# mmurooka/SMPLpp

Hardware: AMD Instinct MI355X
Metric: SMPL FK evals/s + IK iters/s, batch 1024 frames, 1/2/4/8 MI355X (higher is better)
Workload: dtype f32 (exact operands: every fp32 value as three bf16 pieces = fp32's 24 bits on the bf16 matrix pipe, fp32 accumulate; fp32 VALU skinning)

## Files before the change

### smplpp_amd/csrc/ik.hip

```cpp
#include "ik_types.h"
#include "ik_eval.h"
#include "ik_solve.h"
#include "ik_proj.h"
#include "vposer_state.h"

#include <algorithm>
#include <chrono>
#include <cstdlib>

using namespace smplpp_hip;

struct smplpp_ik
{
  smplpp_model * m = nullptr;
  smplpp_vposer * vp = nullptr;
  int64_t n = 0, K = 0;
  int64_t frame_base = 0;
  int theta_dim = TD75;
  TaskArrays ta{};
  float *theta = nullptr, *beta = nullptr, *theta25 = nullptr, *vjac = nullptr;
  float *verts = nullptr, *rest = nullptr, *joints = nullptr, *poserot = nullptr, *pts = nullptr;
  double *e = nullptr, *J = nullptr, *Jl = nullptr, *e2 = nullptr, *xout = nullptr;
  int *skip = nullptr, *status = nullptr, *sticky = nullptr, *list_cnt = nullptr, *list_f = nullptr;
  int * range_word = nullptr;
// ... 343 lines not shown
    HIP_TRY(hipDeviceSynchronize());
    HIP_TRY(hipMemcpy(actual_normal, s->ta.anrm, sizeof(float) * nk * 3, kind));
  }
  return SMPLPP_OK;
}

static int ik_forward_eval(smplpp_ik * s, int optimize_beta, int phi_live, int64_t min_valid, hipStream_t st, hipEvent_t eval_done = nullptr)
{
  smplpp_model * m = s->m;
  const int64_t n = s->n;
  const int K = (int)s->K;
  const float * th25 = s->theta;
  const bool jac_elsewhere = s->vp && s->jac_ahead;
  {
    TraceRange tr_fwd("forward SMPL");
    if(s->vp && s->exact)
    {
      int rc = vposer_jacobian_device(s->vp, s->jxw, n, s->theta + 6, TD44, s->theta25 + 6, 75, s->vjac, st);
      if(rc) return rc;
      th25 = s->theta25;
    }
    else if(s->vp)
    {
      int rc = jac_elsewhere ? vposer_forward_device(s->vp, n, s->theta + 6, TD44, s->theta25 + 6, 75, nullptr, st, s->frame_base, true)
                             : vposer_forward_device(s->vp, n, s->theta + 6, TD44, s->theta25 + 6, 75, s->vjac, st, s->frame_base);
      if(rc) return rc;
      th25 = s->theta25;
    }
    s->vcur ^= 1;
    s->verts = s->vbuf[s->vcur];
    int rc = fk_device(m, n, s->beta, th25, s->verts, s->joints, nullptr, s->rest, s->poserot, st, RANGE_INTERNAL, s->range_word,
                       s->exact ? m->form : 0);
    if(rc) return rc;
  }
  TraceRange tr_eval("calculate IK matrices");
  if(s->side_pending)
  {
    if(s->use_flags)
      HIP_TRY(hipStreamWaitValue32(st, s->sig + 32, s->tick_join, hipStreamWaitValueGte, 0xffffffffu));
    else
      HIP_TRY(hipStreamWaitEvent(st, s->ev_join, 0));
    s->side_pending = false;
  }
  s->jac_ahead = false;
  const bool deep = m->nlev > 9;
  const bool wide = m->madj > MAXADJ;
  const size_t shmem = sizeof(float) * (deep ? (wide ? EvalPlan<DMAX, 64, 3>::L_END : EvalPlan<DMAX, 64, 3>::L_END)
                                             : (wide ? EvalPlan<9, 76, 4>::L_END : EvalPlan<9, 76, 6>::L_END)) + L_ANC_BYTES;
  static PerDeviceOnce once_eval[4];
  const void * kfn = deep ? (wide ? reinterpret_cast<const void *>(&ik_eval_kernel<DMAX, 64, 3, MAXADJ_WIDE>) : reinterpret_cast<const void *>(&ik_eval_kernel<DMAX, 64, 3>))
                          : (wide ? reinterpret_cast<const void *>(&ik_eval_kernel<9, 76, 4, MAXADJ_WIDE>) : reinterpret_cast<const void *>(&ik_eval_kernel<9, 76, 6>));
  HIP_TRY(lds_opt_in(once_eval[(deep ? 1 : 0) + (wide ? 2 : 0)], m->device, kfn, (int)shmem));
  int tsplit = (n < 256) ? (int)(256 / n) : 1;
  if(tsplit > K) tsplit = K;
  if(tsplit < 1) tsplit = 1;
  if(s->use_flags) eval_done = nullptr;
#define EVAL_(DM, RC, NG, MA)                                                                                                              \
  hipExtLaunchKernelGGL((ik_eval_kernel<DM, RC, NG, MA>), dim3((unsigned)(n * tsplit)), dim3(EVAL_NT), shmem, st, nullptr, eval_done, 0,     \
                        view_of(m), s->ta, th25, (const float *)s->verts, (const float *)s->rest, (const float *)m->ws.Gp.as<float>(),     \
                        (const float *)s->joints, (const float *)s->poserot, K, optimize_beta, phi_live, (int)min_valid, s->pts, s->e,     \
                        s->J, s->skip, s->dbg_stop, tsplit, s->roles, s->vp ? (const float *)s->vjac : (const float *)nullptr,             \
                        s->vp ? s->Jl : (double *)nullptr)
  if(deep && wide)
    EVAL_(DMAX, 64, 3, MAXADJ_WIDE);
  else if(deep)
    EVAL_(DMAX, 64, 3, MAXADJ);
  else if(wide)
    EVAL_(9, 76, 4, MAXADJ_WIDE);
  else
    EVAL_(9, 76, 6, MAXADJ);
#undef EVAL_
  HIP_TRY(hipGetLastError());
  s->have_eval = true;
  return SMPLPP_OK;
}

static int ik_check_valence(smplpp_ik * s);

extern "C" int smplpp_ik_eval(smplpp_ik * s, int optimize_beta, double * e, double * J, int space, void * stream)
{
  if(!s) return fail(SMPLPP_ERR_INVALID, "smplpp_ik_eval: null solver");
  int rc = check_space(space, "smplpp_ik_eval");
  if(rc) return rc;
  HIP_TRY(hipSetDevice(s->m->device));
  hipStream_t st = static_cast<hipStream_t>(stream);
  rc = ik_forward_eval(s, optimize_beta, 1, 0, st);
  if(rc) return rc;
  const int64_t D = s->theta_dim + 2 * s->K + (optimize_beta ? NB : 0);
  hipMemcpyKind kind = space == SMPLPP_HOST ? hipMemcpyDeviceToHost : hipMemcpyDeviceToDevice;
  if(e) HIP_TRY(hipMemcpyAsync(e, s->e, sizeof(double) * s->n * s->K * 4, kind, st));
  if(J) HIP_TRY(hipMemcpyAsync(J, s->vp ? s->Jl : s->J, sizeof(double) * s->n * s->K * 4 * D, kind, st));
  if(space == SMPLPP_HOST)
  {
    HIP_TRY(hipStreamSynchronize(st));
    if((rc = ik_check_valence(s))) return rc;
  }
  return SMPLPP_OK;
}

struct SeqHook
{
  float * theta_record = nullptr;
  const float * next_tpos = nullptr;
  const uint8_t * next_valid = nullptr;
  int shared = 0;
};

static int ik_iterate_enqueue(smplpp_ik * s, int iters, int enable_qp, int optimize_beta_from, int64_t min_valid, hipStream_t st,
                              const SeqHook * hook = nullptr, bool more_follows = false)
{
  int rc = SMPLPP_OK;
  smplpp_model * m = s->m;
  const int K = (int)s->K;
  static PerDeviceOnce once_solve[5];
  HIP_TRY(lds_opt_in(once_solve[0], m->device, reinterpret_cast<const void *>(&ik_solve_kernel<false>), (int)SOLVE_LDS_MAX));
  HIP_TRY(lds_opt_in(once_solve[1], m->device, reinterpret_cast<const void *>(&ik_solve_kernel<true>), (int)SOLVE_LDS_MAX));
  HIP_TRY(lds_opt_in(once_solve[2], m->device, reinterpret_cast<const void *>(&ik_solve_kernel<false, 11>), (int)SOLVE_LDS_MAX));
  HIP_TRY(lds_opt_in(once_solve[3], m->device, reinterpret_cast<const void *>(&ik_solve_kernel<false, 5>), (int)SOLVE_LDS_MAX));
  HIP_TRY(lds_opt_in(once_solve[4], m->device, reinterpret_cast<const void *>(&ik_solve_kernel<false, 3>), (int)SOLVE_LDS_MAX));
  if(s->use_flags && (s->tick_fork > 0x7fff0000u || s->tick_join > 0x7fff0000u || s->tick_done > 0x7fff0000u))
  {
    HIP_TRY(hipStreamSynchronize(st));
    HIP_TRY(hipStreamSynchronize(s->side));
    HIP_TRY(hipMemset(s->sig, 0, sizeof(unsigned) * 128));
    s->tick_fork = s->tick_join = s->tick_done = 0;
  }
  const bool dbg = s->dbg_sync;
  const int dbg_stop = s->dbg_stop;
  const bool overlap_ok = s->overlap_ok;
  const int64_t scan_blocks = s->scan_blocks;
#define DBG_SYNC(tag)                                                            \
  if(dbg)                                                                        \
  {                                                                              \
    fprintf(stderr, "[smplpp dbg] it %d: %s ...\n", it, tag);                    \
    HIP_TRY(hipStreamSynchronize(st));                                           \
    fprintf(stderr, "[smplpp dbg] it %d: %s done\n", it, tag);                   \
  }
  for(int it = 0; it < iters; it++)
  {
    const int opt_beta = (optimize_beta_from >= 0 && it >= optimize_beta_from) ? 1 : 0;
    const int phi_live = (optimize_beta_from >= 0) ? (it >= optimize_beta_from ? 1 : 0) : 1;
    const bool beside = overlap_ok && (!phi_live || s->phi_locked);
    rc = ik_forward_eval(s, opt_beta, phi_live, min_valid, st, beside ? s->ev_fork : nullptr);
    if(rc) return rc;
    DBG_SYNC("forward+eval");
    const int beta_dim = opt_beta ? NB : 0;
    const int D = s->theta_dim + 2 * K + beta_dim, rows = 4 * K;
    s->last_D = D;
    const int m_dim = D - ((!phi_live || s->phi_locked) ? 2 * K : 0);
    const int qp_k = (enable_qp && !((!phi_live || s->phi_locked) && beta_dim == 0)) ? 1 : 0;
    const int ntr_primal = (m_dim + 1 <= 48) ? 3 : (m_dim + 1 <= 80) ? 5 : ((m_dim + 1 <= 96 || m_dim + 1 > 176) ? 6 : 11);
    const bool dual_shape = rows < s->theta_dim && rows <= 63 && D <= 192 && dbg_stop != 9;
    const int ntr = dual_shape ? 6 : ntr_primal;
    const size_t fixed = sizeof(double) * ((size_t)(m_dim + 1) * (m_dim + 2) / 2 + 7 * (size_t)D + 2 * (size_t)rows + 128 * (size_t)ntr + 4) + sizeof(int) * 2 * (size_t)D;
    const size_t budget = SOLVE_LDS_MAX;
    int chunk_rows = (int)((budget - fixed) / (sizeof(double) * (size_t)D));
    if(chunk_rows > rows) chunk_rows = rows;
    if(chunk_rows < 4) return fail(SMPLPP_ERR_INVALID, "smplpp_ik_iterate: system too large for the in-LDS solver");
    const size_t solve_shmem = fixed + sizeof(double) * (size_t)chunk_rows * D;
    const bool dual_only = dual_shape && chunk_rows >= rows;
    if(dual_shape && !dual_only) return fail(SMPLPP_ERR_INVALID, "smplpp_ik_iterate: system too large for the in-LDS solver");
    const bool last = hook && it == iters - 1;
    float * theta_record = last ? hook->theta_record : nullptr;
    const bool go = beside && s->use_flags;
    if(go) s->tick_fork++;
    const bool ahead = s->latent_split && go && !opt_beta && (it + 1 < iters || more_follows);
    if(ahead) s->tick_done++;
    unsigned * const done_flag = ahead ? s->sig + 64 : (unsigned *)nullptr;
    unsigned * const done_counter = ahead ? s->sig + 80 : (unsigned *)nullptr;
#define SOLVE_(DO) ik_solve_kernel<DO><<<dim3((unsigned)s->n), dim3(256), solve_shmem, st>>>(                                              \
    s->ta, s->e, s->vp ? s->Jl : s->J, s->theta, s->beta, beside ? nullptr : s->pts, K, s->theta_dim, beta_dim, phi_live, qp_k, \
    s->vp ? 1 : 0, chunk_rows, s->skip, s->e2, s->status, s->sticky, s->xout, dbg_stop, m_dim, s->vp ? s->theta25 : (float *)nullptr, theta_record, \
    go ? s->sig : (unsigned *)nullptr, go ? s->sig + 16 : (unsigned *)nullptr, s->tick_fork, done_flag, done_counter, s->tick_done)
#define SOLVE11_(NTR_) ik_solve_kernel<false, NTR_><<<dim3((unsigned)s->n), dim3(256), solve_shmem, st>>>(                                              \
    s->ta, s->e, s->vp ? s->Jl : s->J, s->theta, s->beta, beside ? nullptr : s->pts, K, s->theta_dim, beta_dim, phi_live, qp_k, \
    s->vp ? 1 : 0, chunk_rows, s->skip, s->e2, s->status, s->sticky, s->xout, dbg_stop, m_dim, s->vp ? s->theta25 : (float *)nullptr, theta_record, \
    go ? s->sig : (unsigned *)nullptr, go ? s->sig + 16 : (unsigned *)nullptr, s->tick_fork, done_flag, done_counter, s->tick_done)
    {
      TraceRange tr_solve("solve IK");
      if(dual_only)
        SOLVE_(true);
      else if(ntr == 11)
        SOLVE11_(11);
      else if(ntr == 5)
        SOLVE11_(5);
      else if(ntr == 3)
        SOLVE11_(3);
      else
        SOLVE_(false);
    }
#undef SOLVE_
#undef SOLVE11_
    HIP_TRY(hipGetLastError());
    DBG_SYNC("solve");
    {
      TraceRange tr_proj("project point");
      const float * qpts = beside ? s->ta.apos : s->pts;
      hipStream_t pst = st;
      if(beside)
      {
        if(s->use_flags)
          HIP_TRY(hipStreamWaitValue32(s->side, s->sig, s->tick_fork, hipStreamWaitValueGte, 0xffffffffu));
        else
          HIP_TRY(hipStreamWaitEvent(s->side, s->ev_fork, 0));
        pst = s->side;
      }
      int chunks = (int)(scan_blocks / s->n);
      chunks = chunks < 1 ? 1 : (chunks > 32 ? 32 : chunks);
      const float * hint = beside ? s->ta.hint : nullptr;
      const dim3 sg((unsigned)(s->n * chunks));
#define SCAN_(KPR, NBT_) proj_scan_kernel<KPR, NBT_><<<sg, dim3(256), 0, pst>>>(view_of(m), s->ta, s->verts, qpts, hint, m->F, K, chunks, s->skip, \
                                                                   s->list_cnt, s->list_d, s->list_f, dbg_stop)
      const bool small_chunk = (m->F + chunks - 1) / chunks <= 3 * 256;
      const bool many = s->scan_form < 0 ? (s->n >= 512 && small_chunk) : s->scan_form == 0;
      if(K <= 8 && many && small_chunk) SCAN_(0, 3);
      else if(K <= 8 && many) SCAN_(0, CP_BATCH);
      else if(K <= 4) SCAN_(2, CP_BATCH);
      else if(K <= 8) SCAN_(4, CP_BATCH);
      else if(small_chunk) SCAN_(0, 3);
      else SCAN_(0, CP_BATCH);
#undef SCAN_
      HIP_TRY(hipGetLastError());
      int *& dbg_buf = s->dbg_buf;
      if(dbg && !dbg_buf) HIP_TRY(dalloc(s, &dbg_buf, 8));
      if(dbg) HIP_TRY(hipMemsetAsync(dbg_buf, 0, sizeof(int) * 8, st));
      int fsplit = (s->n < 256) ? (int)(256 / s->n) : 1;
      if(fsplit > K) fsplit = K;
      if(fsplit < 1) fsplit = 1;
      const bool join_flag = beside && s->use_flags && !ahead;
      if(beside && s->use_flags) s->tick_join++;
      hipExtLaunchKernelGGL(proj_finish_kernel, dim3((unsigned)(s->n * fsplit)), dim3(256), 0, pst, nullptr,
                            (beside && !s->use_flags) ? s->ev_join : nullptr, 0,
                            view_of(m), s->ta, (const float *)s->verts, qpts, m->F, K, (const int *)s->skip, s->list_cnt, s->list_d,
                            s->list_f, dbg ? dbg_buf : (int *)nullptr, fsplit, join_flag ? s->sig + 32 : (unsigned *)nullptr,
                            join_flag ? s->sig + 48 : (unsigned *)nullptr, s->tick_join, last ? hook->next_tpos : (const float *)nullptr,
                            last ? hook->next_valid : (const uint8_t *)nullptr, last ? hook->shared : 0);
      HIP_TRY(hipGetLastError());
      if(ahead)
      {
        HIP_TRY(hipStreamWaitValue32(s->side, s->sig + 64, s->tick_done, hipStreamWaitValueGte, 0xffffffffu));
        rc = vposer_forward_device(s->vp, s->n, s->theta + 6, TD44, nullptr, 75, s->vjac, s->side, s->frame_base, false, s->sig + 32,
                                   s->sig + 48, s->tick_join);
        if(rc) return rc;
        s->jac_ahead = true;
      }
      if(beside) s->side_pending = true;
      if(dbg)
      {
        int h[8];
        HIP_TRY(hipMemcpy(h, dbg_buf, sizeof(h), hipMemcpyDeviceToHost));
        fprintf(stderr, "[smplpp dbg] it %d: project lists: tasks %d, empty %d, overflow %d, nan %d, max cnt %d\n", it, h[0], h[1], h[2], h[3], h[4]);
      }
    }
    DBG_SYNC("project");
  }
#undef DBG_SYNC
  return SMPLPP_OK;
}

static int ik_join(smplpp_ik * s, hipStream_t st)
{
  if(s->side_pending)
  {
    if(s->use_flags)
      HIP_TRY(hipStreamWaitValue32(st, s->sig + 32, s->tick_join, hipStreamWaitValueGte, 0xffffffffu));
    else
      HIP_TRY(hipStreamWaitEvent(st, s->ev_join, 0));
    s->side_pending = false;
  }
  return SMPLPP_OK;
}

static int ik_check_status(smplpp_ik * s, const int * flags)
{
  std::vector<int> h((size_t)s->n);
  HIP_TRY(hipMemcpy(h.data(), flags, sizeof(int) * s->n, hipMemcpyDeviceToHost));
  for(int64_t f = 0; f < s->n; f++)
    if(h[f] & 1) return fail(SMPLPP_ERR_NUMERIC, "LLT has numerical issue!");
  return SMPLPP_OK;
}

static int ik_check_valence(smplpp_ik * s)
{
  std::vector<int> h((size_t)s->n);
  HIP_TRY(hipMemcpy(h.data(), s->sticky, sizeof(int) * s->n, hipMemcpyDeviceToHost));
  for(int64_t f = 0; f < s->n; f++)
    if(h[f] & 4)
      return fail(SMPLPP_ERR_INVALID, "a task with a normal term (normal weight or normal offset) touches a vertex with more than 12 adjacent "
                                      "faces: the Jacobian of such a term is not supported");
  return SMPLPP_OK;
}

extern "C" int smplpp_ik_iterate(smplpp_ik * s, int iters, int enable_qp, int optimize_beta_from, int64_t min_valid,
                                 double * e_sqnorm, int space, void * stream)
{
  if(!s || iters < 0) return fail(SMPLPP_ERR_INVALID, "smplpp_ik_iterate: bad argument");
  int rc = check_space(space, "smplpp_ik_iterate");
  if(rc) return rc;
  HIP_TRY(hipSetDevice(s->m->device));
  hipStream_t st = static_cast<hipStream_t>(stream);
  const auto enq_t0 = std::chrono::steady_clock::now();
  rc = ik_iterate_enqueue(s, iters, enable_qp, optimize_beta_from, min_valid, st);
  s->last_enqueue_us = std::chrono::duration<double, std::micro>(std::chrono::steady_clock::now() - enq_t0).count();
  if(rc)
  {
    (void)ik_join(s, st);
    return rc;
// ... 162 lines not shown
```

### smplpp_amd/csrc/ik_solve.h

```cpp
#pragma once
#include "ik_types.h"

namespace smplpp_hip
{
__device__ inline int tri_idx(int i, int j)
{
  return i * (i + 1) / 2 + j;
}
__device__ inline void tri_unpack(int item, int & i, int & j)
{
  i = (int)((sqrt(8.0 * (double)item + 1.0) - 1.0) * 0.5);
  while(tri_idx(i + 1, 0) <= item) i++;
  while(tri_idx(i, 0) > item) i--;
  j = item - tri_idx(i, 0);
}

__device__ inline void chol_aug(double * M, int nf, int * bad, double * dinv)
{
  const int tid = threadIdx.x, nt = blockDim.x;
  for(int j = 0; j < nf; j++)
  {
    double d = M[tri_idx(j, j)];
    if(!(d > 0.0))
    {
// ... 250 lines not shown
      for(; m + 1 < k; m += 2)
      {
        s -= Li[m] * Lk[m];
        s1 -= Li[m + 1] * Lk[m + 1];
      }
      if(m < k) s -= Li[m] * Lk[m];
      s += s1;
    }
    double piv = readlane_f64(s, k);
    if(!(piv > 0.0))
    {
      badl = true;
      piv = 1.0;
    }
    const double ri = fast_rsqrt(piv);
    if(act && i >= k) M[tri_idx(i, k)] = (i == k) ? piv * ri : s * ri;
    if(i == k) myrinv = ri;
    __builtin_amdgcn_wave_barrier();
    asm volatile("" ::: "memory");
  }
  double yv = (i < r) ? M[tri_idx(r, i)] : 0.0;
  for(int k0 = r - 1; k0 >= 0; k0--)
  {
    const int k = __builtin_amdgcn_readfirstlane(k0);
    const double lk = (i < k) ? M[tri_idx(k, 0) + i] : 0.0;
    const double wk = readlane_f64(yv, k) * readlane_f64(myrinv, k);
    yv = (i == k) ? wk : yv - lk * wk;
  }
  if(i < r) w[i] = yv;
  if(badl && tid == 0) *bad = 1;
}

template<bool PRE>
__device__ __forceinline__ void solve_dual(double * M, const double * __restrict__ J, const double * rowv, double * Jf, const double * diag,
                                           const double * bpri, const int * idx, int nf, int D, int r, double * ginv, double * us, double * w,
                                           double * xs, int * bad, int dbg_stop, const double (&pre)[8], int pre_nf)
{
  const int tid = threadIdx.x;
  const int cnt = r * nf;
  const bool use_pre = PRE && pre_nf == nf && idx[nf - 1] == nf - 1;
  for(int q0 = 0; q0 < cnt; q0 += 256 * 8)
  {
    double t[8];
    if(use_pre && q0 == 0)
    {
#pragma unroll
      for(int u = 0; u < 8; u++) t[u] = pre[u];
    }
    else
#pragma unroll
    for(int u = 0; u < 8; u++)
    {
      int q = q0 + u * 256 + tid;
      q = q < cnt ? q : cnt - 1;
      const int i = q / nf, a = q - i * nf;
      t[u] = J[(int64_t)i * D + idx[a]];
    }
#pragma unroll
    for(int u = 0; u < 8; u++)
    {
      const int q = q0 + u * 256 + tid;
      if(q < cnt) Jf[q] = t[u];
    }
  }
  __syncthreads();
  SOLVE_STAMP(2);
  if(dbg_stop == 31) return;
  if(tid < nf)
  {
    const int a = tid, q = idx[a];
    double c = bpri[q];
    for(int i = 0; i < r; i++) c += Jf[i * nf + a] * rowv[i];
    const double gi = 1.0 / diag[q];
    const double sg = sqrt(gi);
    ginv[a] = gi;
    xs[a] = c * gi;
    us[a] = c * sg;
    for(int i = 0; i < r; i++) Jf[i * nf + a] *= sg;
  }
  __syncthreads();
  SOLVE_STAMP(3);
  if(dbg_stop == 32) return;
  {
    typedef double d4 __attribute__((ext_vector_type(4)));
    const int wave = tid >> 6, l = tid & 63, l16 = l & 15, lq = l >> 4;
    const int ntr = (r + 16) >> 4;
    const int ntile = ntr * (ntr + 1) / 2;
    for(int t = wave; t < ntile; t += 4)
    {
      int ta = 0, tb = t;
      while(tb > ta)
      {
        tb -= ta + 1;
        ta++;
      }
      const int ia = 16 * ta + l16, ib = 16 * tb + l16;
      const double * pa = (ia < r) ? Jf + ia * nf : us;
      const double * pb = Jf + (ib < r ? ib : 0) * nf;
      const bool la = ia <= r, lb = ib < r;
      d4 acc = {0.0, 0.0, 0.0, 0.0};
      for(int k0 = 0; k0 < nf; k0 += 16)
      {
        double a[4], b[4];
#pragma unroll
        for(int u = 0; u < 4; u++)
        {
          const int k = k0 + 4 * u + lq, kk = k < nf ? k : 0;
          a[u] = pa[kk];
          b[u] = pb[kk];
          if(!(la && k < nf)) a[u] = 0.0;
          if(!(lb && k < nf)) b[u] = 0.0;
        }
#pragma unroll
        for(int u = 0; u < 4; u++) acc = __builtin_amdgcn_mfma_f64_16x16x4f64(a[u], b[u], acc, 0, 0, 0);
      }
#pragma unroll
      for(int rr = 0; rr < 4; rr++)
      {
        const int i = 16 * ta + 4 * rr + lq, j = 16 * tb + l16;
        if(i >= j && i <= r && j < r) M[tri_idx(i, j)] = acc[rr] + (i == j ? 1.0 : 0.0);
      }
    }
  }
  __syncthreads();
  SOLVE_STAMP(4);
  if(dbg_stop == 33) return;
  if(tid < 64)
  {
    switch((r + 7) >> 3)
    {
      case 1: chol_wave_reg<8>(M, r, w, bad); break;
      case 2: chol_wave_reg<16>(M, r, w, bad); break;
      case 3:
        if(r == 24)
          chol_wave_reg<24, true>(M, r, w, bad);
        else
          chol_wave_reg<24>(M, r, w, bad);
        break;
      case 4: chol_wave_reg<32>(M, r, w, bad); break;
      default: chol_wave_lds(M, r, w, bad); break;
    }
  }
  __syncthreads();
  SOLVE_STAMP(5);
  if(dbg_stop == 34) return;
  if(tid < nf)
  {
    const int a = tid;
    double t = 0.0;
    for(int i = 0; i < r; i++) t += Jf[i * nf + a] * w[i];
    xs[a] = xs[a] - sqrt(ginv[a]) * t;
  }
  __syncthreads();
}

template<int NT>
__device__ inline void build_and_factor_reg(double * M, const double * __restrict__ J, const double * __restrict__ rowv, double * Jc,
                                            const double * diag, const double * bpri, const int * idx, int nf, int D, int rows,
                                            int chunk_rows, double * lraw , double * ldiag , double * dinv , int * bad,
                                            int dbg_stop, const int * rlist , int nlive)
{
  const int tid = threadIdx.x, tx = tid >> 4, ty = tid & 15;
  double acc[NT][NT];
  typedef double d4 __attribute__((ext_vector_type(4)));
  const int nitemM = (nf + 1) * (nf + 2) / 2;
  const bool ksplit = NT <= 6 && 2 * (NT * (NT + 1) / 2) * 256 + nitemM <= chunk_rows * D;
  if(ksplit)
  {
    constexpr int NTILE = NT <= 6 ? NT * (NT + 1) / 2 : 1, NTK = NT <= 6 ? NT : 1;
    const int wave = tid >> 6, l = tid & 63, l16 = l & 15, lq = l >> 4;
    d4 tacc[NTILE];
    int colT[NTK];
#pragma unroll
    for(int t = 0; t < NTK; t++)
    {
      const int m = 16 * t + l16;
      colT[t] = (m < nf) ? idx[m] : (m == nf ? -1 : -2);
    }
#pragma unroll
    for(int u = 0; u < NTILE; u++) tacc[u] = d4{0.0, 0.0, 0.0, 0.0};
    const int W = nf > 0 ? idx[nf - 1] + 1 : 1;
    const bool whole = W == D && nlive == rows;
    const int Weven = W + (W & 1);
    const int crows_dma = dma_chunk_rows(chunk_rows, D, Weven);
    const bool dma = !whole && W < D && crows_dma >= 4 && (int64_t)rows * D * 8 < 0x7fffff00LL;
    const int Wp = dma ? Weven : W;
    const int crows = dma ? crows_dma : (int)(((int64_t)chunk_rows * D) / W);
    if(dbg_stop == 40) return;
    SOLVE_STAMP(2);
    for(int c0 = 0; c0 < nlive; c0 += crows)
    {
      const int cr = (nlive - c0 < crows) ? nlive - c0 : crows;
      __syncthreads();
      SOLVE_STAMP(3);
      if(whole)
        stage_rows(Jc, J + (int64_t)c0 * D, cr * D);
      else if(dma)
        stage_rows_cols_dma(Jc, J, cr, W, D, rlist + c0, rows);
      else
        stage_rows_cols(Jc, J, cr, W, D, rlist + c0);
      SOLVE_STAMP(4);
      __syncthreads();
      SOLVE_STAMP(5);
      if(dbg_stop == 41) return;
      for(int r0 = 4 * wave; r0 < cr; r0 += 16)
      {
        const int r = r0 + lq;
        const bool rin = r < cr;
        const double rv = rowv[rlist[c0 + (rin ? r : 0)]];
        const double * Jr = Jc + (rin ? r : 0) * Wp;
        double v[NTK], va[NTK], vb[NTK];
#pragma unroll
        for(int t = 0; t < NTK; t++) v[t] = Jr[colT[t] >= 0 ? colT[t] : 0];
#pragma unroll
        for(int t = 0; t < NTK; t++)
        {
          va[t] = !rin ? 0.0 : (colT[t] >= 0 ? v[t] : (colT[t] == -1 ? rv : 0.0));
          vb[t] = (rin && colT[t] >= 0) ? v[t] : 0.0;
        }
#pragma unroll
        for(int ta = 0; ta < NTK; ta++)
#pragma unroll
          for(int tb = 0; tb <= ta; tb++)
          {
            if(!(16 * ta <= nf && 16 * tb < nf)) continue;
            d4 & t = tacc[ta * (ta + 1) / 2 + tb];
            t = __builtin_amdgcn_mfma_f64_16x16x4f64(va[ta], vb[tb], t, 0, 0, 0);
          }
      }
    }
    __syncthreads();
    SOLVE_STAMP(6);
    if(dbg_stop == 42) return;
    constexpr int PRAW = NTILE * 4 * 64;
    double * const praw = Jc + (size_t)((wave & 1) * PRAW);
    double * const ptri = Jc + 2 * PRAW;
    if(wave >= 2)
    {
#pragma unroll
      for(int u = 0; u < NTILE; u++)
#pragma unroll
        for(int rr = 0; rr < 4; rr++) praw[(u * 4 + rr) * 64 + l] = tacc[u][rr];
    }
    __syncthreads();
    if(wave < 2)
    {
#pragma unroll
      for(int u = 0; u < NTILE; u++)
#pragma unroll
        for(int rr = 0; rr < 4; rr++) tacc[u][rr] += praw[(u * 4 + rr) * 64 + l];
      double * P = wave == 0 ? M : ptri;
#pragma unroll
      for(int ta = 0; ta < NTK; ta++)
#pragma unroll
        for(int tb = 0; tb <= ta; tb++)
        {
          if(!(16 * ta <= nf && 16 * tb < nf)) continue;
#pragma unroll
          for(int rr = 0; rr < 4; rr++)
          {
            const int i = 16 * ta + 4 * rr + lq, k = 16 * tb + l16;
            if(i >= k && i <= nf && k < nf) P[tri_idx(i, k)] = tacc[ta * (ta + 1) / 2 + tb][rr];
          }
        }
    }
    __syncthreads();
#pragma unroll
    for(int a2 = 0; a2 < NT; a2++)
#pragma unroll
      for(int b2 = 0; b2 <= a2; b2++)
      {
        const int i = ty + 16 * a2, k = tx + 16 * b2;
        double sum = 0.0;
        if(i >= k && i <= nf && k < nf)
        {
          const int q = tri_idx(i, k);
          sum = M[q] + ptri[q];
        }
        acc[a2][b2] = sum;
      }
    __syncthreads();
  }
  else
  {
    constexpr int NTILE = NT * (NT + 1) / 2, TPW = (NTILE + 3) / 4;
    const int wave = tid >> 6, l = tid & 63, l16 = l & 15, lq = l >> 4;
    d4 tacc[TPW];
    int colA[TPW], colB[TPW];
    bool live[TPW];
#pragma unroll
    for(int u = 0; u < TPW; u++)
    {
      const int t = wave + 4 * u;
      int ta = 0, tb = t;
      while(tb > ta)
      {
        tb -= ta + 1;
        ta++;
      }
      live[u] = t < NTILE && 16 * ta <= nf && 16 * tb < nf;
      const int mi = 16 * ta + l16, mk = 16 * tb + l16;
      colA[u] = (mi < nf) ? idx[mi] : (mi == nf ? -1 : -2);
      colB[u] = (mk < nf) ? idx[mk] : -2;
      tacc[u] = d4{0.0, 0.0, 0.0, 0.0};
    }
    const int W = nf > 0 ? idx[nf - 1] + 1 : 1;
    const bool whole = W == D && nlive == rows;
    const int Weven = W + (W & 1);
    const int crows_dma = dma_chunk_rows(chunk_rows, D, Weven);
    const bool dma = !whole && W < D && crows_dma >= 4 && (int64_t)rows * D * 8 < 0x7fffff00LL;
    const int Wp = dma ? Weven : W;
    const int crows = dma ? crows_dma : (int)(((int64_t)chunk_rows * D) / W);
    if(dbg_stop == 40) return;
    SOLVE_STAMP(2);
    for(int c0 = 0; c0 < nlive; c0 += crows)
    {
      const int cr = (nlive - c0 < crows) ? nlive - c0 : crows;
      __syncthreads();
      SOLVE_STAMP(3);
      if(whole)
        stage_rows(Jc, J + (int64_t)c0 * D, cr * D);
      else if(dma)
        stage_rows_cols_dma(Jc, J, cr, W, D, rlist + c0, rows);
      else
        stage_rows_cols(Jc, J, cr, W, D, rlist + c0);
      SOLVE_STAMP(4);
      __syncthreads();
      SOLVE_STAMP(5);
      if(dbg_stop == 41) return;
      for(int r0 = 0; r0 < cr; r0 += 4)
      {
        const int r = r0 + lq;
        const bool rin = r < cr;
        const double rv = rowv[rlist[c0 + (rin ? r : 0)]];
        const double * Jr = Jc + (rin ? r : 0) * Wp;
        double ja[TPW], jb[TPW];
#pragma unroll
        for(int u = 0; u < TPW; u++)
        {
          ja[u] = Jr[colA[u] >= 0 ? colA[u] : 0];
          jb[u] = Jr[colB[u] >= 0 ? colB[u] : 0];
        }
#pragma unroll
        for(int u = 0; u < TPW; u++)
        {
          if(!live[u]) continue;
          const double va = !rin ? 0.0 : (colA[u] >= 0 ? ja[u] : (colA[u] == -1 ? rv : 0.0));
          const double vb = (rin && colB[u] >= 0) ? jb[u] : 0.0;
          tacc[u] = __builtin_amdgcn_mfma_f64_16x16x4f64(va, vb, tacc[u], 0, 0, 0);
        }
      }
    }
    __syncthreads();
    SOLVE_STAMP(6);
    if(dbg_stop == 42) return;
#pragma unroll
    for(int u = 0; u < TPW; u++)
    {
      if(!live[u]) continue;
      const int t = wave + 4 * u;
      int ta = 0, q = t;
      while(q > ta)
      {
        q -= ta + 1;
        ta++;
      }
      const int tb = q;
#pragma unroll
      for(int rr = 0; rr < 4; rr++)
      {
        const int i = 16 * ta + 4 * rr + lq, k = 16 * tb + l16;
        if(i >= k && i <= nf && k < nf) M[tri_idx(i, k)] = tacc[u][rr];
      }
    }
    __syncthreads();
#pragma unroll
    for(int a2 = 0; a2 < NT; a2++)
#pragma unroll
      for(int b2 = 0; b2 <= a2; b2++)
      {
        const int i = ty + 16 * a2, k = tx + 16 * b2;
        acc[a2][b2] = (i >= k && i <= nf && k < nf) ? M[tri_idx(i, k)] : 0.0;
      }
    __syncthreads();
  }
  {
    const int ar = nf >> 4;
    int id_[NT], ib_[NT];
#pragma unroll
    for(int a = 0; a < NT; a++)
    {
      const int i = ty + 16 * a, k = tx + 16 * a;
      id_[a] = idx[(ty == tx && i < nf) ? i : 0];
      ib_[a] = idx[k < nf ? k : 0];
    }
    double dv[NT], bv[NT];
#pragma unroll
    for(int a = 0; a < NT; a++)
    {
      dv[a] = diag[id_[a]];
      bv[a] = bpri[ib_[a]];
    }
#pragma unroll
    for(int a = 0; a < NT; a++)
    {
      const int i = ty + 16 * a;
      acc[a][a] += (ty == tx && i < nf) ? dv[a] : 0.0;
#pragma unroll
      for(int b = 0; b <= a; b++)
        acc[a][b] += (a == ar && i == nf && tx + 16 * b < nf) ? bv[b] : 0.0;
    }
  }
  if(dbg_stop == 4) return;
  SOLVE_STAMP(7);
  constexpr int LS = 16 * NT;
  bool kcol[NT];
#pragma unroll
  for(int a = 0; a < NT; a++) kcol[a] = tx + 16 * a < nf;
  for(int q = tid; q < 8 * LS; q += 256) lraw[q] = 0.0;
  __syncthreads();
  int par = 0;
#pragma unroll
  for(int bj = 0; bj < NT; bj++)
  {
    for(int jj = 0; jj < 16; jj += 4)
    {
      const int j0 = 16 * bj + jj;
      if(j0 >= nf) break;
      const int ncol = nf - j0 < 4 ? nf - j0 : 4;
      double * lb = lraw + (par & 1) * 4 * LS;
      par++;
      if(tx >= jj && tx < jj + ncol)
      {
        double * lp = lb + (tx - jj) * LS;
        const int jc = j0 + (tx - jj);
#pragma unroll
        for(int a = bj; a < NT; a++)
        {
          const int i = ty + 16 * a;
          if(i >= jc && i <= nf) lp[i] = acc[a][bj];
        }
      }
      __syncthreads();
      double inv[4], L[4][4];
      {
        double Cj[4][4];
#pragma unroll
        for(int sidx = 0; sidx < 4; sidx++)
        {
#pragma unroll
          for(int q = sidx; q < 4; q++)
          {
            double v = (q < ncol) ? lb[sidx * LS + j0 + q] : 0.0;
#pragma unroll
            for(int t = 0; t < sidx; t++) v -= Cj[t][q] * L[sidx][t];
            Cj[sidx][q] = v;
          }
          double d = Cj[sidx][sidx];
          if(sidx < ncol && !(d > 0.0)) *bad = 1;
          if(!(sidx < ncol && d > 0.0)) d = 1.0;
          double r = __builtin_amdgcn_rcp(d);
          r = r * (2.0 - d * r);
          r = r * (2.0 - d * r);
          inv[sidx] = (sidx < ncol) ? r : 0.0;
#pragma unroll
          for(int q = sidx + 1; q < 4; q++) L[q][sidx] = (q < ncol) ? Cj[sidx][q] * inv[sidx] : 0.0;
        }
      }
      double ri[4][NT], sk[4][NT];
#pragma unroll
      for(int a = bj; a < NT; a++)
      {
        const int i = ty + 16 * a, k = tx + 16 * a;
        double ci[4], ck[4];
#pragma unroll
        for(int q = 0; q < 4; q++)
        {
          double vi = lb[q * LS + i], vk = lb[q * LS + k];
#pragma unroll
          for(int t = 0; t < q; t++)
          {
            vi -= ci[t] * L[q][t];
            vk -= ck[t] * L[q][t];
          }
          ci[q] = (a > bj || i > j0 + q) ? vi : 0.0;
          ck[q] = (a > bj || k > j0 + q) ? vk : 0.0;
          ri[q][a] = (q < ncol) ? ci[q] : 0.0;
          sk[q][a] = (q < ncol && kcol[a]) ? ck[q] * inv[q] : 0.0;
        }
      }
#pragma unroll
      for(int a = bj; a < NT; a++)
#pragma unroll
        for(int b = bj; b <= a; b++)
          acc[a][b] -= (ri[0][a] * sk[0][b] + ri[1][a] * sk[1][b]) + (ri[2][a] * sk[2][b] + ri[3][a] * sk[3][b]);
    }
  }
  __syncthreads();
  SOLVE_STAMP(8);
#pragma unroll
  for(int a = 0; a < NT; a++)
  {
    const int i = ty + 16 * a;
    if(ty == tx && i < nf)
    {
      double d = acc[a][a];
      if(!(d > 0.0))
      {
        *bad = 1;
        d = 1.0;
      }
      dinv[i] = fast_rsqrt(d);
    }
  }
  __syncthreads();
#pragma unroll
  for(int a = 0; a < NT; a++)
#pragma unroll
    for(int b = 0; b <= a; b++)
    {
      const int i = ty + 16 * a, k = tx + 16 * b;
      if(k < nf && i >= k && i <= nf) M[tri_idx(i, k)] = acc[a][b] * dinv[k];
    }
  __syncthreads();
}

template<bool DUAL_ONLY, int NTR = 6>
__global__ __launch_bounds__(256) void ik_solve_kernel(TaskArrays ta, const double * __restrict__ e_all, const double * __restrict__ J_all,
                                                       float * __restrict__ theta, float * __restrict__ beta, float * __restrict__ pts,
                                                       int K, int theta_dim, int beta_dim, int phi_live, int enable_qp, int use_prior,
                                                       int chunk_rows, const int * __restrict__ skip, double * __restrict__ e2_out,
                                                       int * __restrict__ status, int * __restrict__ sticky, double * __restrict__ x_out, int dbg_stop, int m_dim,
                                                       float * __restrict__ theta25, float * __restrict__ theta_copy,
                                                       unsigned * __restrict__ go_flag, unsigned * __restrict__ go_counter, unsigned go_tick,
                                                       unsigned * __restrict__ done_flag, unsigned * __restrict__ done_counter, unsigned done_tick)
{
  extern __shared__ __attribute__((aligned(16))) double sm[];
  const int64_t f = blockIdx.x;
  const int tid = threadIdx.x;
  SOLVE_STAMP(0);
  if(go_flag && tid == 0)
  {
    if(__hip_atomic_fetch_add(go_counter, 1u, __ATOMIC_RELAXED, __HIP_MEMORY_SCOPE_AGENT) == gridDim.x - 1)
    {
      __hip_atomic_store(go_counter, 0u, __ATOMIC_RELAXED, __HIP_MEMORY_SCOPE_AGENT);
      __hip_atomic_store(go_flag, go_tick, __ATOMIC_RELAXED, __HIP_MEMORY_SCOPE_SYSTEM);
    }
  }
  const int D = theta_dim + 2 * K + beta_dim, rows = 4 * K;
  const int64_t tb = f * K;
  double * M = sm;
  double * Jc = M + (m_dim + 1) * (m_dim + 2) / 2;
  double * xs = Jc + chunk_rows * D;
  double * xfull = xs + D;
  double * diag = xfull + D;
  double * bpri = diag + D;
  double * lo = bpri + D;
  double * hi = lo + D;
  double * rowv = hi + D;
  double * lraw = rowv + rows;
  double * ldiag = lraw + 128 * NTR;
  double * dinv = ldiag + 4;
  int * idx = reinterpret_cast<int *>(dinv + D);
  int * state = idx + D;
  double * ebuf = reinterpret_cast<double *>(state + D);
  __shared__ int s_bad, s_nf, s_block, s_bside, s_done, s_anybound, s_wcnt[4], s_wany[4];
  __shared__ int s_rlist[DUAL_ONLY ? 1 : IK_MAXK * 4], s_nlive;
  __shared__ double s_alpha, s_e2;
  const double * J = J_all + f * rows * (int64_t)D;
  const int skipf = skip[f];
  double e_pre[(IK_MAXK * 4 + 255) / 256];
#pragma unroll
  for(int u = 0; u < (IK_MAXK * 4 + 255) / 256; u++) e_pre[u] = (tid + 256 * u < rows) ? e_all[f * rows + tid + 256 * u] : 0.0;
  const int my_i = tid < D ? tid : 0;
  const bool my_phi = my_i >= theta_dim && my_i < theta_dim + 2 * K;
  const float pl_pre = (D <= 256 && my_phi && phi_live) ? ta.philim[tb + (my_i - theta_dim) / 2] : 0.0f;
  const float th_pre = (D <= 256 && use_prior && my_i < theta_dim) ? theta[f * theta_dim + my_i] : 0.0f;
  float rl_pre[(IK_MAXK * 4 + 63) / 64];
  if constexpr(!DUAL_ONLY)
  {
#pragma unroll
    for(int c = 0; c < (IK_MAXK * 4 + 63) / 64; c++)
    {
      const int r = 64 * c + (tid & 63), k = (r < rows ? r : 0) >> 2;
      rl_pre[c] = ta.roww[(tb + k) * 2 + (((r & 3) == 3) ? 1 : 0)];
    }
  }
  double j_pre[8];
  if constexpr(DUAL_ONLY)
  {
    const int cnt = rows * theta_dim;
#pragma unroll
    for(int u = 0; u < 8; u++)
    {
      int q = u * 256 + tid;
      q = q < cnt ? q : cnt - 1;
      const int i = q / theta_dim, a = q - i * theta_dim;
      j_pre[u] = J[(int64_t)i * D + a];
    }
  }
  if(skipf)
  {
    if(tid == 0 && e2_out) e2_out[f] = 0.0;
    if(pts)
      for(int k = tid; k < K * 3; k += 256) pts[tb * 3 + k] = ta.apos[tb * 3 + k];
    if(theta_copy)
      for(int i = tid; i < theta_dim; i += 256) theta_copy[f * theta_dim + i] = theta[f * theta_dim + i];
    wg_signal(done_flag, done_counter, done_tick);
    return;
  }
  __builtin_amdgcn_s_setprio(3);
#pragma unroll
  for(int u = 0; u < (IK_MAXK * 4 + 255) / 256; u++)
    if(tid + 256 * u < rows) ebuf[tid + 256 * u] = e_pre[u];
  __syncthreads();
  const double * e = ebuf;
  if(tid < 64)
  {
    double v[3];
#pragma unroll
    for(int a = 0; a < 3; a++) v[a] = (tid + 64 * a < rows) ? e[tid + 64 * a] : 0.0;
    double s = 0.0;
    if(rows <= 192)
    {
      s = v[0] * v[0];
      s = fma(v[1], v[1], s);
      s = fma(v[2], v[2], s);
#pragma unroll
      for(int o = 32; o > 0; o >>= 1) s += __shfl_xor(s, o, 64);
    }
    else
      for(int r = 0; r < rows; r++) s += e[r] * e[r];
    if(tid == 0)
    {
      s_e2 = s;
      s_bad = (sticky[f] & 4) ? 1 : 0;
      s_done = 0;
      if(e2_out) e2_out[f] = s;
    }
  }
  else if(!DUAL_ONLY && tid < 128)
  {
    const int l = tid - 64;
    int base = 0;
#pragma unroll
    for(int c = 0; c < (IK_MAXK * 4 + 63) / 64; c++)
    {
      const int r = 64 * c + l;
      const bool lv = r < rows && (((r & 3) == 3) ? (rl_pre[c] > 0.0f) : (rl_pre[c] != 0.0f));
      const unsigned long long m = __ballot(lv);
      if(lv) s_rlist[base + __popcll(m & ((1ull << l) - 1ull))] = r;
      base += __popcll(m);
    }
    if(l == 0) s_nlive = base;
  }
  __syncthreads();
  for(int i = tid; i < D; i += 256)
  {
    const double reg = (i < theta_dim) ? 1e-3 : (i < theta_dim + 2 * K ? 1e-1 : 1e-3);
    double dg = reg + s_e2;
    double bp = 0.0;
    if(use_prior && i < theta_dim)
    {
      const double w = (i < 6) ? 0.0 : (i >= theta_dim - 6 ? 1e3 : 1e-5);
      dg += w;
      bp = w * (double)(D <= 256 ? th_pre : theta[f * theta_dim + i]);
    }
    diag[i] = dg;
    bpri[i] = bp;
    double l = -1e30, h = 1e30;
    int st = 0;
    if(i >= theta_dim && i < theta_dim + 2 * K)
    {
      const double pl = phi_live ? (double)(D <= 256 ? pl_pre : ta.philim[tb + (i - theta_dim) / 2]) : 0.0;
      if(enable_qp)
      {
        l = -pl;
        h = pl;
      }
      if(!(pl > 0.0))
      {
        l = 0.0;
        h = 0.0;
        st = 2;
      }
    }
    else if(i >= theta_dim + 2 * K && enable_qp)
    {
      l = -0.5;
      h = 0.5;
    }
    lo[i] = l;
    hi[i] = h;
    state[i] = st;
    xfull[i] = 0.0;
  }
  __syncthreads();

  SOLVE_STAMP(1);
  if(dbg_stop == 1) return;
  const int max_it = enable_qp ? 4 * D + 20 : 1;
  for(int it = 0; it < max_it; it++)
  {
    if(D <= 256)
    {
      int st = 2;
      if(tid < D) st = state[tid];
      const int is_free = (st == 0), is_b = ((st == -1 || st == 1) && xfull[tid < D ? tid : 0] != 0.0);
      const uint64_t m = __ballot(is_free);
      const int wave = tid >> 6, lane = tid & 63;
      const uint64_t mbnd = __ballot(is_b);
      if(lane == 0)
      {
        s_wcnt[wave] = __popcll(m);
// ... 299 lines not shown
```

### smplpp_amd/csrc/ik_types.h

```cpp
#pragma once
#include "mesh_device.h"
#include "staging.h"
#include "trace.h"
#include "signal.h"

#include <hip/hip_ext.h>

struct smplpp_vposer;

namespace smplpp_hip
{
int fk_device(smplpp_model * m, int64_t n, const float * beta, const float * theta, float * verts, float * joints,
              float * xforms44, float * rest, float * poserot, hipStream_t st, int range_slot, int * range_word = nullptr,
              char form_override = 0);
int vposer_forward_device(smplpp_vposer * v, int64_t n, const float * z, int64_t z_stride, float * out, int64_t out_stride,
                          float * jac, hipStream_t st, int64_t frame_base, bool value_like_jac = false, unsigned * sig_flag = nullptr,
                          unsigned * sig_counter = nullptr, unsigned sig_tick = 0u);

constexpr int TD75 = SMPLPP_THETA_DIM;
constexpr int TD44 = SMPLPP_LATENT_POSE_DIM;
constexpr int NQ = TD75 + NB;
constexpr int IK_MAXK = 48;
constexpr size_t SOLVE_LDS_MAX = 160 * 1024 - 1536;
constexpr int MAXD = TD75 + 2 * IK_MAXK + NB;

struct TaskArrays
{
  int32_t * face;
  float * vw;
  float * tang;
  float * tpos;
  float * tnrm;
  float * posw;
  float * nrmw;
  float * philim;
  float * noff;
  float * apos;
  float * anrm;
  float * hint;
  int * flags;
  float * roww;
};

struct ModelView
{
  const int32_t * faces;
  const int32_t * adjOff;
  const int32_t * adjFace;
  const int32_t * parent;
  const uint8_t * wIdx;
  const float * wVal;
  const float * wSum;
  const float * Pvm;
  const float * Svm;
  const float * JS;
  const uint16_t * faceRing;
  const uint8_t * faceMap;
  const int32_t * anc;
  int nlev;
  int64_t V;
  int maxw;
};

__device__ inline void lds_barrier()
{
  asm volatile("s_waitcnt lgkmcnt(0)\n\ts_barrier" ::: "memory");
}

#ifndef SMPLPP_EVAL_NT
#define SMPLPP_EVAL_NT 768
#endif
constexpr int EVAL_NT = SMPLPP_EVAL_NT;
#ifdef SMPLPP_EVAL_STAMPS
__device__ unsigned long long g_eval_stamps[64 * 16];
#define EVAL_STAMP(i) do { if(tid == 0 && blockIdx.x < 64) g_eval_stamps[blockIdx.x * 16 + (i)] = __builtin_readcyclecounter(); } while(0)
#else
#define EVAL_STAMP(i) do {} while(0)
#endif
#ifdef SMPLPP_SOLVE_STAMPS
__device__ unsigned long long g_solve_stamps[64 * 16];
#define SOLVE_STAMP(i) do { if(threadIdx.x == 0 && blockIdx.x < 64) g_solve_stamps[blockIdx.x * 16 + (i)] = __builtin_amdgcn_s_memrealtime(); } while(0)
#else
#define SOLVE_STAMP(i) do {} while(0)
#endif
}
```

Baseline: 15.02 million.

## Factor Cholesky in 16-column panels with one wave, overlapping trailing updates

For the 3- and 5-tile register-resident Cholesky, the 4-column step loop is replaced by a blocked scheme. One wave factors each 16-column panel in registers using readlane broadcasts, while the other threads apply the previous panel's rank-16 update to the trailing tiles. Panel buffers are double-buffered in LDS with a padded stride, which cuts the number of block barriers per factorization. The LDS budget accounting is extended, and static asserts guard the larger panel scratch, which may lower chunk_rows.

```diff
diff --git a/smplpp_amd/csrc/ik.hip b/smplpp_amd/csrc/ik.hip
--- a/smplpp_amd/csrc/ik.hip
+++ b/smplpp_amd/csrc/ik.hip
@@ -519,7 +519,7 @@
     const int ntr_primal = (m_dim + 1 <= 48) ? 3 : (m_dim + 1 <= 80) ? 5 : ((m_dim + 1 <= 96 || m_dim + 1 > 176) ? 6 : 11);
     const bool dual_shape = rows < s->theta_dim && rows <= 63 && D <= 192 && dbg_stop != 9;
     const int ntr = dual_shape ? 6 : ntr_primal;
-    const size_t fixed = sizeof(double) * ((size_t)(m_dim + 1) * (m_dim + 2) / 2 + 7 * (size_t)D + 2 * (size_t)rows + 128 * (size_t)ntr + 4) + sizeof(int) * 2 * (size_t)D;
+    const size_t fixed = solve_lds_fixed(m_dim, D, rows, ntr);
     const size_t budget = SOLVE_LDS_MAX;
     int chunk_rows = (int)((budget - fixed) / (sizeof(double) * (size_t)D));
     if(chunk_rows > rows) chunk_rows = rows;
diff --git a/smplpp_amd/csrc/ik_solve.h b/smplpp_amd/csrc/ik_solve.h
--- a/smplpp_amd/csrc/ik_solve.h
+++ b/smplpp_amd/csrc/ik_solve.h
@@ -426,6 +426,81 @@
     xs[a] = xs[a] - sqrt(ginv[a]) * t;
   }
   __syncthreads();
+}
+
+template<int NC, bool R2>
+__device__ __forceinline__ void panel_factor_wave(double * Cp, double * invp, int nrows, int ncol, int * bad)
+{
+  typedef double d2 __attribute__((ext_vector_type(2)));
+  constexpr int PS = PANEL_PS;
+  const int l = threadIdx.x;
+  const bool in0 = l < nrows, in1 = R2 && l + 64 < nrows;
+  double r0[16], r1[R2 ? 16 : 1];
+  {
+    const d2 * p0 = reinterpret_cast<const d2 *>(Cp + (in0 ? l : 0) * PS);
+#pragma unroll
+    for(int u = 0; u < 8; u++)
+    {
+      const d2 v = p0[u];
+      r0[2 * u] = (in0 && l >= 2 * u) ? v.x : 0.0;
+      r0[2 * u + 1] = (in0 && l >= 2 * u + 1) ? v.y : 0.0;
+    }
+    if constexpr(R2)
+    {
+      const d2 * p1 = reinterpret_cast<const d2 *>(Cp + (in1 ? l + 64 : 0) * PS);
+#pragma unroll
+      for(int u = 0; u < 8; u++)
+      {
+        const d2 v = p1[u];
+        r1[2 * u] = in1 ? v.x : 0.0;
+        r1[2 * u + 1] = in1 ? v.y : 0.0;
+      }
+    }
+  }
+  bool badl = false;
+  double myinv = 0.0;
+#pragma unroll
+  for(int k = 0; k < 16; k++)
+  {
+    if(NC ? k < NC : k < ncol)
+    {
+      double d = readlane_f64(r0[k], k);
+      if(!(d > 0.0))
+      {
+        badl = true;
+        d = 1.0;
+      }
+      double r = __builtin_amdgcn_rcp(d);
+      r = r * (2.0 - d * r);
+      r = r * (2.0 - d * r);
+      const double sl = r0[k] * r;
+      if(l == k) myinv = r;
+#pragma unroll
+      for(int j = k + 1; j < (NC ? NC : 16); j++)
+      {
+        const double x = readlane_f64(sl, j);
+        r0[j] = fma(-r0[k], x, r0[j]);
+        if constexpr(R2) r1[j] = fma(-r1[k], x, r1[j]);
+      }
+    }
+  }
+  if(in0)
+  {
+    d2 * p0 = reinterpret_cast<d2 *>(Cp + l * PS);
+#pragma unroll
+    for(int u = 0; u < 8; u++) p0[u] = d2{r0[2 * u], r0[2 * u + 1]};
+  }
+  if constexpr(R2)
+  {
+    if(in1)
+    {
+      d2 * p1 = reinterpret_cast<d2 *>(Cp + (l + 64) * PS);
+#pragma unroll
+      for(int u = 0; u < 8; u++) p1[u] = d2{r1[2 * u], r1[2 * u + 1]};
+    }
+  }
+  if(l < 16) invp[l] = (l < (NC ? NC : ncol)) ? myinv : 0.0;
+  if(badl && l == 0) *bad = 1;
 }
 
 template<int NT>
@@ -687,87 +762,183 @@
   }
   if(dbg_stop == 4) return;
   SOLVE_STAMP(7);
-  constexpr int LS = 16 * NT;
-  bool kcol[NT];
-#pragma unroll
-  for(int a = 0; a < NT; a++) kcol[a] = tx + 16 * a < nf;
-  for(int q = tid; q < 8 * LS; q += 256) lraw[q] = 0.0;
-  __syncthreads();
-  int par = 0;
-#pragma unroll
-  for(int bj = 0; bj < NT; bj++)
-  {
-    for(int jj = 0; jj < 16; jj += 4)
-    {
-      const int j0 = 16 * bj + jj;
-      if(j0 >= nf) break;
-      const int ncol = nf - j0 < 4 ? nf - j0 : 4;
-      double * lb = lraw + (par & 1) * 4 * LS;
-      par++;
-      if(tx >= jj && tx < jj + ncol)
-      {
-        double * lp = lb + (tx - jj) * LS;
-        const int jc = j0 + (tx - jj);
-#pragma unroll
+  if constexpr(solve_panelled(NT))
+  {
+    typedef double d2 __attribute__((ext_vector_type(2)));
+    constexpr int PS = PANEL_PS, PB = 16 * NT * PS;
+    double * const cb0 = lraw + ((reinterpret_cast<uintptr_t>(lraw) >> 3) & 1);
+    double * const invb = cb0 + 2 * PB;
+    const int wave = tid >> 6;
+    bool kcol[NT];
+#pragma unroll
+    for(int a = 0; a < NT; a++) kcol[a] = tx + 16 * a < nf;
+    auto publish = [&](int b) {
+      double * cb = cb0 + (b & 1) * PB;
+#pragma unroll
+      for(int a = 0; a < NT; a++)
+        if(a >= b) cb[(ty + 16 * a) * PS + tx] = acc[a][b];
+    };
+    auto apply = [&](int q, int blo, int bhi) {
+      const double * cb = cb0 + (q & 1) * PB;
+      const double * iv = invb + (q & 1) * 16;
+#pragma unroll
+      for(int s0 = 0; s0 < 16; s0 += 4)
+      {
+        if(16 * q + s0 >= nf) break;
+        const d2 i01 = *reinterpret_cast<const d2 *>(iv + s0), i23 = *reinterpret_cast<const d2 *>(iv + s0 + 2);
+        double ri[NT][4], sk[NT][4];
+#pragma unroll
+        for(int a = 0; a < NT; a++)
+        {
+          if(a < blo) continue;
+          const d2 * pr = reinterpret_cast<const d2 *>(cb + (ty + 16 * a) * PS + s0);
+          const d2 v01 = pr[0], v23 = pr[1];
+          ri[a][0] = v01.x;
+          ri[a][1] = v01.y;
+          ri[a][2] = v23.x;
+          ri[a][3] = v23.y;
+          if(a >= bhi) continue;
+          const d2 * pc = reinterpret_cast<const d2 *>(cb + (tx + 16 * a) * PS + s0);
+          const d2 c01 = pc[0], c23 = pc[1];
+          sk[a][0] = kcol[a] ? c01.x * i01.x : 0.0;
+          sk[a][1] = kcol[a] ? c01.y * i01.y : 0.0;
+          sk[a][2] = kcol[a] ? c23.x * i23.x : 0.0;
+          sk[a][3] = kcol[a] ? c23.y * i23.y : 0.0;
+        }
+#pragma unroll
+        for(int a = 0; a < NT; a++)
+#pragma unroll
+          for(int b = 0; b <= a; b++)
+            if(b >= blo && b < bhi) acc[a][b] -= (ri[a][0] * sk[b][0] + ri[a][1] * sk[b][1]) + (ri[a][2] * sk[b][2] + ri[a][3] * sk[b][3]);
+      }
+    };
+    publish(0);
+    __syncthreads();
+#pragma unroll
+    for(int p = 0; p < NT; p++)
+    {
+      if(16 * p >= nf) break;
+      const int ncol = nf - 16 * p < 16 ? nf - 16 * p : 16;
+      double * cb = cb0 + (p & 1) * PB;
+      if(wave == 0)
+      {
+        double * Cp = cb + 16 * p * PS;
+        double * ip = invb + (p & 1) * 16;
+        constexpr int nrows_max = 16 * NT;
+        const int nrows = nrows_max - 16 * p;
+        if(nrows > 64)
+        {
+          if(ncol == 16)
+            panel_factor_wave<16, (nrows_max > 64)>(Cp, ip, nrows, ncol, bad);
+          else
+            panel_factor_wave<0, (nrows_max > 64)>(Cp, ip, nrows, ncol, bad);
+        }
+        else if(ncol == 16)
+          panel_factor_wave<16, false>(Cp, ip, nrows, ncol, bad);
+        else if(ncol == 11)
+          panel_factor_wave<11, false>(Cp, ip, nrows, ncol, bad);
+        else if(ncol == 12)
+          panel_factor_wave<12, false>(Cp, ip, nrows, ncol, bad);
+        else
+          panel_factor_wave<0, false>(Cp, ip, nrows, ncol, bad);
+      }
+      if(p > 0) apply(p - 1, p + 1, NT);
+      __syncthreads();
+#pragma unroll
+      for(int a = 0; a < NT; a++)
+        if(a >= p) acc[a][p] = cb[(ty + 16 * a) * PS + tx];
+      if(p + 1 < NT && 16 * (p + 1) < nf)
+      {
+        apply(p, p + 1, p + 2);
+        publish(p + 1);
+        __syncthreads();
+      }
+    }
+  }
+  else
+  {
+    constexpr int LS = 16 * NT;
+    bool kcol[NT];
+  #pragma unroll
+    for(int a = 0; a < NT; a++) kcol[a] = tx + 16 * a < nf;
+    for(int q = tid; q < 8 * LS; q += 256) lraw[q] = 0.0;
+    __syncthreads();
+    int par = 0;
+  #pragma unroll
+    for(int bj = 0; bj < NT; bj++)
+    {
+      for(int jj = 0; jj < 16; jj += 4)
+      {
+        const int j0 = 16 * bj + jj;
+        if(j0 >= nf) break;
+        const int ncol = nf - j0 < 4 ? nf - j0 : 4;
+        double * lb = lraw + (par & 1) * 4 * LS;
+        par++;
+        if(tx >= jj && tx < jj + ncol)
+        {
+          double * lp = lb + (tx - jj) * LS;
+          const int jc = j0 + (tx - jj);
+  #pragma unroll
+          for(int a = bj; a < NT; a++)
+          {
+            const int i = ty + 16 * a;
+            if(i >= jc && i <= nf) lp[i] = acc[a][bj];
+          }
+        }
+        __syncthreads();
+        double inv[4], L[4][4];
+        {
+          double Cj[4][4];
+  #pragma unroll
+          for(int sidx = 0; sidx < 4; sidx++)
+          {
+  #pragma unroll
+            for(int q = sidx; q < 4; q++)
+            {
+              double v = (q < ncol) ? lb[sidx * LS + j0 + q] : 0.0;
+  #pragma unroll
+              for(int t = 0; t < sidx; t++) v -= Cj[t][q] * L[sidx][t];
+              Cj[sidx][q] = v;
+            }
+            double d = Cj[sidx][sidx];
+            if(sidx < ncol && !(d > 0.0)) *bad = 1;
+            if(!(sidx < ncol && d > 0.0)) d = 1.0;
+            double r = __builtin_amdgcn_rcp(d);
+            r = r * (2.0 - d * r);
+            r = r * (2.0 - d * r);
+            inv[sidx] = (sidx < ncol) ? r : 0.0;
+  #pragma unroll
+            for(int q = sidx + 1; q < 4; q++) L[q][sidx] = (q < ncol) ? Cj[sidx][q] * inv[sidx] : 0.0;
+          }
+        }
+        double ri[4][NT], sk[4][NT];
+  #pragma unroll
         for(int a = bj; a < NT; a++)
         {
-          const int i = ty + 16 * a;
-          if(i >= jc && i <= nf) lp[i] = acc[a][bj];
-        }
-      }
-      __syncthreads();
-      double inv[4], L[4][4];
-      {
-        double Cj[4][4];
-#pragma unroll
-        for(int sidx = 0; sidx < 4; sidx++)
-        {
-#pragma unroll
-          for(int q = sidx; q < 4; q++)
+          const int i = ty + 16 * a, k = tx + 16 * a;
+          double ci[4], ck[4];
+  #pragma unroll
+          for(int q = 0; q < 4; q++)
           {
-            double v = (q < ncol) ? lb[sidx * LS + j0 + q] : 0.0;
-#pragma unroll
-            for(int t = 0; t < sidx; t++) v -= Cj[t][q] * L[sidx][t];
-            Cj[sidx][q] = v;
+            double vi = lb[q * LS + i], vk = lb[q * LS + k];
+  #pragma unroll
+            for(int t = 0; t < q; t++)
+            {
+              vi -= ci[t] * L[q][t];
+              vk -= ck[t] * L[q][t];
+            }
+            ci[q] = (a > bj || i > j0 + q) ? vi : 0.0;
+            ck[q] = (a > bj || k > j0 + q) ? vk : 0.0;
+            ri[q][a] = (q < ncol) ? ci[q] : 0.0;
+            sk[q][a] = (q < ncol && kcol[a]) ? ck[q] * inv[q] : 0.0;
           }
-          double d = Cj[sidx][sidx];
-          if(sidx < ncol && !(d > 0.0)) *bad = 1;
-          if(!(sidx < ncol && d > 0.0)) d = 1.0;
-          double r = __builtin_amdgcn_rcp(d);
-          r = r * (2.0 - d * r);
-          r = r * (2.0 - d * r);
-          inv[sidx] = (sidx < ncol) ? r : 0.0;
-#pragma unroll
-          for(int q = sidx + 1; q < 4; q++) L[q][sidx] = (q < ncol) ? Cj[sidx][q] * inv[sidx] : 0.0;
-        }
-      }
-      double ri[4][NT], sk[4][NT];
-#pragma unroll
-      for(int a = bj; a < NT; a++)
-      {
-        const int i = ty + 16 * a, k = tx + 16 * a;
-        double ci[4], ck[4];
-#pragma unroll
-        for(int q = 0; q < 4; q++)
-        {
-          double vi = lb[q * LS + i], vk = lb[q * LS + k];
-#pragma unroll
-          for(int t = 0; t < q; t++)
-          {
-            vi -= ci[t] * L[q][t];
-            vk -= ck[t] * L[q][t];
-          }
-          ci[q] = (a > bj || i > j0 + q) ? vi : 0.0;
-          ck[q] = (a > bj || k > j0 + q) ? vk : 0.0;
-          ri[q][a] = (q < ncol) ? ci[q] : 0.0;
-          sk[q][a] = (q < ncol && kcol[a]) ? ck[q] * inv[q] : 0.0;
-        }
-      }
-#pragma unroll
-      for(int a = bj; a < NT; a++)
-#pragma unroll
-        for(int b = bj; b <= a; b++)
-          acc[a][b] -= (ri[0][a] * sk[0][b] + ri[1][a] * sk[1][b]) + (ri[2][a] * sk[2][b] + ri[3][a] * sk[3][b]);
+        }
+  #pragma unroll
+        for(int a = bj; a < NT; a++)
+  #pragma unroll
+          for(int b = bj; b <= a; b++)
+            acc[a][b] -= (ri[0][a] * sk[0][b] + ri[1][a] * sk[1][b]) + (ri[2][a] * sk[2][b] + ri[3][a] * sk[3][b]);
+      }
     }
   }
   __syncthreads();
@@ -833,7 +1004,7 @@
   double * hi = lo + D;
   double * rowv = hi + D;
   double * lraw = rowv + rows;
-  double * ldiag = lraw + 128 * NTR;
+  double * ldiag = lraw + solve_lraw_doubles(NTR);
   double * dinv = ldiag + 4;
   int * idx = reinterpret_cast<int *>(dinv + D);
   int * state = idx + D;
diff --git a/smplpp_amd/csrc/ik_types.h b/smplpp_amd/csrc/ik_types.h
--- a/smplpp_amd/csrc/ik_types.h
+++ b/smplpp_amd/csrc/ik_types.h
@@ -23,6 +23,24 @@
 constexpr int IK_MAXK = 48;
 constexpr size_t SOLVE_LDS_MAX = 160 * 1024 - 1536;
 constexpr int MAXD = TD75 + 2 * IK_MAXK + NB;
+
+constexpr bool solve_panelled(int ntr)
+{
+  return ntr == 3 || ntr == 5;
+}
+constexpr int PANEL_PS = 18;
+constexpr int solve_lraw_doubles(int ntr)
+{
+  return solve_panelled(ntr) ? 2 * 16 * ntr * PANEL_PS + 32 + 2 : 128 * ntr;
+}
+static_assert(solve_lraw_doubles(3) >= 256 && solve_lraw_doubles(5) >= 256, "solve_dual's vectors live in the same block");
+constexpr size_t solve_lds_fixed(int m_dim, int D, int rows, int ntr)
+{
+  return sizeof(double) * ((size_t)(m_dim + 1) * (m_dim + 2) / 2 + 7 * (size_t)D + 2 * (size_t)rows + (size_t)solve_lraw_doubles(ntr) + 4)
+         + sizeof(int) * 2 * (size_t)D;
+}
+static_assert(solve_lds_fixed(47, 47 + 2 * IK_MAXK, 4 * IK_MAXK, 3) + sizeof(double) * 4 * (47 + 2 * IK_MAXK) <= SOLVE_LDS_MAX, "LDS plan, 3 tiles");
+static_assert(solve_lds_fixed(79, 79 + 2 * IK_MAXK, 4 * IK_MAXK, 5) + sizeof(double) * 4 * (79 + 2 * IK_MAXK) <= SOLVE_LDS_MAX, "LDS plan, 5 tiles");
 
 struct TaskArrays
 {
```

Result: no change. 14.98 million (median of 2 runs) (-0.3%).
